# nicrie/xmca

Hardware: AMD Instinct MI355X
Metric: MCA solve+rotate throughput (ms_per_step = solve+rotate wall-clock, ms); rule_n surrogates/s in `rule_n` (higher is better)
Workload: dtype f64; 1 GPU; C2: synthetic EOF T=2920 x N=10000 float64 (generator A), solve() + rotate(n_rot=10, power=1); parallelism=replicas x1 (solve/rotate do not shard); rule_n run-sharded x1

## Files before the change

### xmca_amd/csrc/tridiag.h

```cpp
#pragma once
#include <algorithm>
#include <cmath>
#include <cstring>
#include <vector>

#include "common.h"

namespace xmca {

constexpr int TRD_THREADS = 512;
constexpr int TRD_ROWS = 4;
constexpr int TRD_MAX_WGS = 256;
constexpr int TRD_MAX_ITERS = 32;

struct TrdParams {
  double* Ar;
  double* Ai;
  int64_t ld;
  int n;
  double* vb[2][2];
  double* pb[2][2];
  double* gp[2][2];
  double* tau[2];
  double* d;
// ... 657 lines not shown
      if (is_writer && tid == 0) P.d[j] = dj_sh;
      break;
    }
    const double a0r = a0_sh[cur][0], a0i = CPLX ? a0_sh[cur][1] : 0.0;
    double beta, tr, ti = 0.0, scr = 0.0, sci = 0.0;
    if (xn2 == 0.0 && a0i == 0.0) {
      beta = a0r;
      tr = 0.0;
    } else {
      beta = -copysign(trd_sqrt(a0r * a0r + a0i * a0i + xn2), a0r);
      const double rb = trd_rcp(beta);
      tr = fma(fma(-(beta - a0r) * rb, beta, beta - a0r), rb, (beta - a0r) * rb);
      ti = -a0i * rb;
      const double dr = a0r - beta, di = a0i, dn = trd_rcp(dr * dr + di * di);
      scr = dr * dn;
      sci = -di * dn;
    }
    const double mr_ = trd_uniform(tr * scr - ti * sci), mi_ = trd_uniform(tr * sci + ti * scr);
    const double tr_next = trd_uniform(tr), ti_next = trd_uniform(ti), sr_next = trd_uniform(scr), si_next = trd_uniform(sci);
    if (is_writer && tid == 0) {
      P.d[j] = dj_sh;
      P.e[j] = beta;
      P.tau[0][j] = tr;
      if (CPLX) P.tau[1][j] = ti;
    }
    if (prof) P.prof[8 * j + 3] = __builtin_amdgcn_s_memtime();
    const int g0 = ((j + 1) >> 7) / CG;
    const int c0 = (j + 1) >> 7;
    if (lane == 0) bX[0][j + 1] = a0r - beta;
    const unsigned int tgn = trd_tag_of(j + 1);
    double* const xnext = reinterpret_cast<double*>(reinterpret_cast<char*>(S.xch) + xwr);
    auto publish_p = [&](int i, double pr, double pi) {
      if constexpr (CPLX) {
        trd_st16_sc1(S.xch, xbytes, 16 * i, xwr + xhalf, trd_tagged(pr, tgn), trd_tagged(pi, tgn));
      } else {
        trd_st_sc1(xnext + 2 * i + 1, trd_tagged(pr, tgn));
      }
    };
    {
      constexpr int MC = (NC + 3) / 4;
      int i = (int)blockIdx.x;
      if (i < j + 1) i += ((j + 1 - i + nwg - 1) / nwg) * nwg;
      int par = 0;
      for (; i < first_res; i += nwg, par ^= 1) {
        const double svr_ = bV[0][i], swr_ = bW[0][i];
        const double svi_ = CPLX ? bV[1][i] : 0.0, swi_ = CPLX ? bW[1][i] : 0.0;
        double* rowr = P.Ar + (int64_t)i * P.ld;
        double* rowi = CPLX ? P.Ai + (int64_t)i * P.ld : nullptr;
        double sr = 0.0, si = 0.0;
        const bool pubrow = i == j + 1;
#pragma unroll 1
        for (int u0 = 0; u0 < MC; u0 += 4) {
        double2 la[4], lb[4];
#pragma unroll
        for (int uu = 0; uu < 4; ++uu) {
          const int u = u0 + uu;
          const int c = u < MC ? c0 + wave + 4 * u : NC;
          la[uu] = make_double2(0.0, 0.0);
          lb[uu] = make_double2(0.0, 0.0);
          if (c < NC) {
            la[uu] = *reinterpret_cast<const double2*>(rowr + 128 * c + 2 * lane);
            if (CPLX) lb[uu] = *reinterpret_cast<const double2*>(rowi + 128 * c + 2 * lane);
          }
        }
#pragma unroll
        for (int uu = 0; uu < 4; ++uu) {
          const int u = u0 + uu;
          const int c = u < MC ? c0 + wave + 4 * u : NC;
          if (c < NC) {
            const int k = 128 * c + 2 * lane;
            double2 a = la[uu];
            const double2 wk = *reinterpret_cast<const double2*>(bW[0] + k);
            const double2 vk = *reinterpret_cast<const double2*>(bV[0] + k);
            const double2 xk = *reinterpret_cast<const double2*>(bX[0] + k);
            if (CPLX) {
              double2 b = lb[uu];
              const double2 wki = *reinterpret_cast<const double2*>(bW[1] + k);
              const double2 vki = *reinterpret_cast<const double2*>(bV[1] + k);
              const double2 xki = *reinterpret_cast<const double2*>(bX[1] + k);
              a.x -= (svr_ * wk.x + svi_ * wki.x) + (swr_ * vk.x + swi_ * vki.x);
              b.x -= (svi_ * wk.x - svr_ * wki.x) + (swi_ * vk.x - swr_ * vki.x);
              a.y -= (svr_ * wk.y + svi_ * wki.y) + (swr_ * vk.y + swi_ * vki.y);
              b.y -= (svi_ * wk.y - svr_ * wki.y) + (swi_ * vk.y - swr_ * vki.y);
              *reinterpret_cast<double2*>(rowr + k) = a;
              *reinterpret_cast<double2*>(rowi + k) = b;
              sr += a.x * xk.x - b.x * xki.x;
              si += a.x * xki.x + b.x * xk.x;
              sr += a.y * xk.y - b.y * xki.y;
              si += a.y * xki.y + b.y * xk.y;
              if (pubrow) {
                trd_st16_sc1(S.xch, xbytes, 16 * k, xwr, trd_tagged(a.x, tgn), trd_tagged(b.x, tgn));
                trd_st16_sc1(S.xch, xbytes, 16 * k + 16, xwr, trd_tagged(a.y, tgn), trd_tagged(b.y, tgn));
              }
            } else {
              a.x -= svr_ * wk.x + swr_ * vk.x;
              a.y -= svr_ * wk.y + swr_ * vk.y;
              *reinterpret_cast<double2*>(rowr + k) = a;
              sr += a.x * xk.x;
              sr += a.y * xk.y;
            }
            if (pubrow) {
              if constexpr (!CPLX) {
                trd_st_sc1(xnext + 2 * k, trd_tagged(a.x, tgn));
                trd_st_sc1(xnext + 2 * k + 2, trd_tagged(a.y, tgn));
              }
            }
          }
        }
        }
        sr = trd_wave_sum_dpp(sr);
        if (CPLX) si = trd_wave_sum_dpp(si);
        if (lane == 0) {
          rowpart[par][wave][0] = sr;
          rowpart[par][wave][1] = si;
        }
        __syncthreads();
        if (wave == 0) {
          const double yr = ((rowpart[par][0][0] + rowpart[par][1][0]) + rowpart[par][2][0]) + rowpart[par][3][0];
          const double yi = CPLX ? ((rowpart[par][0][1] + rowpart[par][1][1]) + rowpart[par][2][1]) + rowpart[par][3][1] : 0.0;
          const double pr = mr_ * yr - mi_ * yi, pi = mr_ * yi + mi_ * yr;
          if (lane == 0) publish_p(i, pr, pi);
        }
      }
    }
    if (rowi[RR - 1] > j) {
      double vpr[RR], vpi[RR], wpr[RR], wpi[RR], accr[RR], acci[RR];
#pragma unroll
      for (int t = 0; t < RR; ++t) {
        const int i = rowi[t];
        const int ii = i < n ? i : 0;
        vpr[t] = i < n ? bV[0][ii] : 0.0; wpr[t] = i < n ? bW[0][ii] : 0.0;
        vpi[t] = (CPLX && i < n) ? bV[1][ii] : 0.0; wpi[t] = (CPLX && i < n) ? bW[1][ii] : 0.0;
        accr[t] = 0.0; acci[t] = 0.0;
      }
#pragma unroll
      for (int cg = 0; cg < NC / CG; ++cg) {
        if (cg >= g0) {
#pragma unroll
          for (int cc = 0; cc < CG; ++cc) {
            const int c = cg * CG + cc;
            const int k = 128 * c + 2 * lane;
            const double2 wk = *reinterpret_cast<const double2*>(bW[0] + k);
            const double2 vk = *reinterpret_cast<const double2*>(bV[0] + k);
            const double2 xk = *reinterpret_cast<const double2*>(bX[0] + k);
            double2 wki = make_double2(0.0, 0.0), vki = wki, xki = wki;
            if (CPLX) {
              wki = *reinterpret_cast<const double2*>(bW[1] + k);
              vki = *reinterpret_cast<const double2*>(bV[1] + k);
              xki = *reinterpret_cast<const double2*>(bX[1] + k);
            }
#pragma unroll
            for (int t = 0; t < RR; ++t) {
              double2 a = ar[t][c];
              if (CPLX) {
                double2 b = ai[t][c];
                a.x = fma(-vpr[t], wk.x, a.x);  a.x = fma(-vpi[t], wki.x, a.x);  a.x = fma(-wpr[t], vk.x, a.x);  a.x = fma(-wpi[t], vki.x, a.x);
                b.x = fma(-vpi[t], wk.x, b.x);  b.x = fma(vpr[t], wki.x, b.x);   b.x = fma(-wpi[t], vk.x, b.x);  b.x = fma(wpr[t], vki.x, b.x);
                a.y = fma(-vpr[t], wk.y, a.y);  a.y = fma(-vpi[t], wki.y, a.y);  a.y = fma(-wpr[t], vk.y, a.y);  a.y = fma(-wpi[t], vki.y, a.y);
                b.y = fma(-vpi[t], wk.y, b.y);  b.y = fma(vpr[t], wki.y, b.y);   b.y = fma(-wpi[t], vk.y, b.y);  b.y = fma(wpr[t], vki.y, b.y);
                ai[t][c] = b;
                accr[t] = fma(a.x, xk.x, accr[t]);  accr[t] = fma(-b.x, xki.x, accr[t]);
                acci[t] = fma(a.x, xki.x, acci[t]); acci[t] = fma(b.x, xk.x, acci[t]);
                accr[t] = fma(a.y, xk.y, accr[t]);  accr[t] = fma(-b.y, xki.y, accr[t]);
                acci[t] = fma(a.y, xki.y, acci[t]); acci[t] = fma(b.y, xk.y, acci[t]);
              } else {
                a.x = fma(-vpr[t], wk.x, a.x);  a.x = fma(-wpr[t], vk.x, a.x);
                a.y = fma(-vpr[t], wk.y, a.y);  a.y = fma(-wpr[t], vk.y, a.y);
                accr[t] = fma(a.x, xk.x, accr[t]);
                accr[t] = fma(a.y, xk.y, accr[t]);
              }
              ar[t][c] = a;
            }
          }
          __builtin_amdgcn_sched_barrier(0);
        }
      }
#pragma unroll
      for (int t = 0; t < RR; ++t) {
        if (rowi[t] == j + 1) {
          int lane2 = 2 * lane;
          asm volatile("" : "+v"(lane2));
#pragma unroll
          for (int c = 0; c < NC; ++c) {
            if (c >= c0) {
              const int k = 128 * c + lane2;
              if constexpr (CPLX) {
                trd_st16_sc1(S.xch, xbytes, 16 * k, xwr, trd_tagged(ar[t][c].x, tgn), trd_tagged(ai[t][c].x, tgn));
                trd_st16_sc1(S.xch, xbytes, 16 * k + 16, xwr, trd_tagged(ar[t][c].y, tgn), trd_tagged(ai[t][c].y, tgn));
              } else {
                trd_st_sc1(xnext + 2 * k, trd_tagged(ar[t][c].x, tgn));
                trd_st_sc1(xnext + 2 * k + 2, trd_tagged(ar[t][c].y, tgn));
              }
            }
          }
        }
      }
      if (j + 1 == j_end && j_end < n) {
#pragma unroll
        for (int t = 0; t < RR; ++t) {
          if (rowi[t] > j && rowi[t] < n) {
            int lane2 = 2 * lane;
            asm volatile("" : "+v"(lane2));
            double* const dr_ = P.Ar + (int64_t)rowi[t] * P.ld;
            double* const di_ = CPLX ? P.Ai + (int64_t)rowi[t] * P.ld : nullptr;
#pragma unroll
            for (int c = 0; c < NC; ++c) {
              if (c >= c0) {
                const int k = 128 * c + lane2;
                *reinterpret_cast<double2*>(dr_ + k) = ar[t][c];
                if (CPLX) *reinterpret_cast<double2*>(di_ + k) = ai[t][c];
              }
            }
          }
        }
      }
#pragma unroll
      for (int t = 0; t < RR; ++t) {
        const int i = rowi[t];
        if (i < n && i > j) {
          const double yr = trd_wave_sum_dpp(accr[t]);
          const double yi = CPLX ? trd_wave_sum_dpp(acci[t]) : 0.0;
          const double pr = mr_ * yr - mi_ * yi, pi = mr_ * yi + mi_ * yr;
          if (lane == 0) publish_p(i, pr, pi);
        }
      }
    }
    if (prof) P.prof[8 * j + 4] = __builtin_amdgcn_s_memtime();
    __syncthreads();
    if (prof) P.prof[8 * j + 6] = __builtin_amdgcn_s_memtime();
    if (give_up_sh) {
      if (tid == 0) atomicExch(S.give_up, 1);
      break;
    }
    if (is_writer && j + 1 == j_end && j_end < n) {
      int s0 = tid;
      asm volatile("" : "+v"(s0));
      for (int s = s0; s < LV; s += TRD_RES_THREADS) {
        S.hand_u[0][s] = bX[0][s];
        if (CPLX) S.hand_u[1][s] = bX[1][s];
      }
      if (tid == 0) {
        S.hand_s[0] = tr_next; S.hand_s[1] = ti_next; S.hand_s[2] = sr_next; S.hand_s[3] = si_next;
      }
    }
    { double* t0 = bV[0]; bV[0] = bX[0]; bX[0] = t0; }
    if (CPLX) { double* t1 = bV[1]; bV[1] = bX[1]; bX[1] = t1; }
    tpr = tr_next;
    tpi = ti_next;
    spr = sr_next;
    spi = si_next;
  }
}

__global__ void trd_prefill_kernel(const double* __restrict__ Wr, const double* __restrict__ Wi, int n, double* __restrict__ xch) {
  const int k = blockIdx.x * blockDim.x + threadIdx.x;
  if (k >= n) return;
  if (Wi) {
    xch[2 * k] = trd_untagged(Wr[k]);
    xch[2 * k + 1] = trd_untagged(Wi[k]);
  } else {
    xch[2 * k] = trd_untagged(Wr[k]);
  }
}

__global__ __launch_bounds__(256) void trd_maxabs_kernel(const double* __restrict__ Ar, const double* __restrict__ Ai, int n, int64_t lda,
                                                         unsigned long long* __restrict__ acc) {
  double m = 0.0;
  bool bad = false;
  for (int r = blockIdx.x; r < n; r += gridDim.x)
    for (int c = threadIdx.x; c < n; c += 256) {
      const double a = fabs(Ar[(int64_t)r * lda + c]), b = Ai ? fabs(Ai[(int64_t)r * lda + c]) : 0.0;
      if (!(a <= 1.7e308) || !(b <= 1.7e308)) bad = true;
      m = fmax(m, fmax(a, b));
    }
  for (int o = 32; o > 0; o >>= 1) m = fmax(m, __shfl_xor(m, o));
  if (__any(bad)) { if ((threadIdx.x & 63) == 0) atomicOr(acc + 1, 1ull); }
  else if ((threadIdx.x & 63) == 0 && m > 0.0) atomicMax(acc, (unsigned long long)__double_as_longlong(m));
}
__global__ void trd_scale_kernel(const unsigned long long* __restrict__ acc, double* __restrict__ scal) {
  const double g = __longlong_as_double((long long)acc[0]);
  const bool nan = acc[1] != 0ull;
  double f = 1.0;
  if (g > 0.0 && !nan) {
    int ex;
    frexp(g, &ex);
    f = ldexp(1.0, -ex);
  }
  scal[0] = f;
  scal[1] = nan ? 1.0 : 0.0;
}

__global__ void trd_copy_kernel(const double* __restrict__ Ar, const double* __restrict__ Ai, int n, int64_t lda, double* Wr, double* Wi,
                                int64_t ld, const double* __restrict__ scal) {
  const double f = scal[0];
  const int r = blockIdx.x;
  for (int c = threadIdx.x; c < ld; c += blockDim.x) {
    const bool in = c < n;
    Wr[(int64_t)r * ld + c] = in ? f * Ar[(int64_t)r * lda + c] : 0.0;
    if (Wi) Wi[(int64_t)r * ld + c] = in ? f * Ai[(int64_t)r * lda + c] : 0.0;
  }
}

constexpr int TRD_BIS_THREADS = 256;
__global__ __launch_bounds__(TRD_BIS_THREADS) void trd_bisect_kernel(const double* __restrict__ d, const double* __restrict__ e, int n,
                                                                   const double* __restrict__ scal, double* lam_desc, double* lam_asc_scaled, int* flag) {
  extern __shared__ __attribute__((aligned(16))) double bis_lds[];
  __shared__ double red[2][TRD_BIS_THREADS / 64];
  double* sd = bis_lds;
  double* se2 = bis_lds + n;
  const int tid = threadIdx.x;
  double gl = 1.7e308, gu = -1.7e308;
  bool bad = false;
  for (int i = tid; i < n; i += TRD_BIS_THREADS) {
    const double di = d[i];
    const double el = i > 0 ? e[i - 1] : 0.0, er = i < n - 1 ? e[i] : 0.0;
    if (!(fabs(di) <= 1.7e308) || !(fabs(er) <= 1.7e308)) bad = true;
    sd[i] = di;
    se2[i] = fmax(er * er, 0x1p-200);
    const double r = fabs(el) + fabs(er);
    gl = fmin(gl, di - r);
    gu = fmax(gu, di + r);
  }
  for (int o = 32; o > 0; o >>= 1) {
    gl = fmin(gl, __shfl_xor(gl, o));
    gu = fmax(gu, __shfl_xor(gu, o));
  }
  if (__any(bad) && flag) { if ((tid & 63) == 0) atomicOr(flag, 1); }
  if ((tid & 63) == 0) { red[0][tid >> 6] = gl; red[1][tid >> 6] = gu; }
  __syncthreads();
  for (int w = 0; w < TRD_BIS_THREADS / 64; ++w) { gl = fmin(gl, red[0][w]); gu = fmax(gu, red[1][w]); }
  const double bnorm = fmax(fabs(gl), fabs(gu));
  gl -= 2.2e-16 * bnorm * n + 1e-300;
  gu += 2.2e-16 * bnorm * n + 1e-300;
  const int grp = tid >> 4, l = tid & 15;
  const int k = blockIdx.x * (TRD_BIS_THREADS / 16) + grp;
  const bool live = k < n;
  double lo = gl, hi = gu;
  const int gshift = ((tid & 63) >> 4) * 16;
  for (int pass = 0; pass < 14; ++pass) {
    const double x = lo + (hi - lo) * ((double)(l + 1) * (1.0 / 17.0));
    double pm = 1.0, pc = sd[0] - x;
    unsigned int sc = (unsigned int)__double2hiint(pc);
    int cnt = (int)(sc >> 31);
    int i = 1;
    double dv[8], ev[8];
    if (i + 8 <= n) {
#pragma unroll
      for (int u = 0; u < 8; ++u) { dv[u] = sd[i + u]; ev[u] = se2[i + u - 1]; }
    }
    for (; i + 8 <= n; i += 8) {
      double dn[8], en[8];
      const int inext = i + 16 <= n ? i + 8 : i;
#pragma unroll
      for (int u = 0; u < 8; ++u) { dn[u] = sd[inext + u]; en[u] = se2[inext + u - 1]; }
#pragma unroll
      for (int u = 0; u < 8; ++u) {
        const double pn = fma(dv[u] - x, pc, -(ev[u] * pm));
        const unsigned int sn = (unsigned int)__double2hiint(pn);
        cnt += (int)((sn ^ sc) >> 31);
        sc = sn;
        pm = pc;
        pc = pn;
      }
      const double mx = fmax(fabs(pc), fabs(pm));
      if (mx == 0.0) pc = (sc >> 31) ? -1.0 : 1.0;
      const int ex = __builtin_amdgcn_frexp_exp(mx);
      pc = ldexp(pc, -ex);
      pm = ldexp(pm, -ex);
#pragma unroll
      for (int u = 0; u < 8; ++u) { dv[u] = dn[u]; ev[u] = en[u]; }
    }
    for (; i < n; ++i) {
      const double pn = fma(sd[i] - x, pc, -(se2[i - 1] * pm));
      const unsigned int sn = (unsigned int)__double2hiint(pn);
      cnt += (int)((sn ^ sc) >> 31);
      sc = sn;
      pm = pc;
      pc = pn;
    }
    const unsigned long long mask = __ballot(cnt <= k);
    const int s = __popcll((mask >> gshift) & 0xFFFFull);
    const double x_lo = __shfl(x, s > 0 ? s - 1 : 0, 16);
    const double x_hi = __shfl(x, s < 16 ? s : 15, 16);
    if (s > 0) lo = x_lo;
    if (s < 16) hi = x_hi;
  }
  if (live && l == 0) {
    lam_desc[n - 1 - k] = 0.5 * (lo + hi) / scal[0];
    if (lam_asc_scaled) lam_asc_scaled[k] = 0.5 * (lo + hi);
  }
}

struct TrdWorkspace {
  DevBuf<double> W[2];
  DevBuf<double> V[2];
  DevBuf<double> vec;
  DevBuf<double> scal;
  DevBuf<int> flag;
  DevBuf<unsigned long long> prof;
  DevBuf<double> sync;
  DevBuf<unsigned int> flags;
  int resident_used = 0;
  int stages_used = 0;
  std::string last_desc;
  hipEvent_t ev[2] = {nullptr, nullptr};
  bool ev_pending = false;
  double reduce_ms = 0.0;
  long long reduce_calls = 0;
  long long resident_calls = 0;
  void ev_begin(hipStream_t st) {
    if (!ev[0]) { XMCA_HIP(hipEventCreate(&ev[0])); XMCA_HIP(hipEventCreate(&ev[1])); }
    XMCA_HIP(hipEventRecord(ev[0], st));
  }
  void ev_end(hipStream_t st) { XMCA_HIP(hipEventRecord(ev[1], st)); ev_pending = true; }
  void ev_collect() {
    if (!ev_pending) return;
    float t = 0.f;
    if (hipEventSynchronize(ev[1]) == hipSuccess && hipEventElapsedTime(&t, ev[0], ev[1]) == hipSuccess) { reduce_ms += t; ++reduce_calls; }
    ev_pending = false;
  }
  ~TrdWorkspace() { if (ev[0]) { (void)hipEventDestroy(ev[0]); (void)hipEventDestroy(ev[1]); } }
  double ms = 0.0;
};

inline bool trd_enabled() {
  const char* e = std::getenv("XMCA_TRIDIAG");
  return !(e && e[0] == '0');
}

inline size_t trd_step_lds(int n, bool cplx) { return (size_t)(((n + 3) + 1) & ~1) * 3 * (cplx ? 2 : 1) * sizeof(double); }

inline bool trd_fits(int n, bool cplx) {
  return trd_step_lds(n, cplx) + 8192 <= (size_t)160 * 1024 && n + 4 <= 16 * TRD_THREADS && (size_t)n * 16 <= (size_t)150 * 1024;
}

struct TrdLayout {
  int n;
  int64_t ld;
  size_t nv;
  double* base;
  TrdParams params(double* Wr, double* Wi, double* Vr, double* Vi) const {
    TrdParams P{};
    P.Ar = Wr; P.Ai = Wi; P.ld = ld; P.n = n;
    double* p = base;
    for (int a = 0; a < 2; ++a) for (int c = 0; c < 2; ++c) { P.vb[a][c] = p; p += nv; }
    for (int a = 0; a < 2; ++a) for (int c = 0; c < 2; ++c) { P.pb[a][c] = p; p += nv; }
    for (int a = 0; a < 2; ++a) for (int c = 0; c < 2; ++c) { P.gp[a][c] = p; p += TRD_MAX_WGS; }
    for (int c = 0; c < 2; ++c) { P.tau[c] = p; p += nv; }
    P.d = p; p += nv;
    P.e = p; p += nv;
    P.Vr = Vr; P.Vi = Vi;
    P.prof = nullptr;
    return P;
  }
  static size_t doubles(size_t nv) { return nv * 12 + (size_t)TRD_MAX_WGS * 8; }
};


inline int trd_resident_nc(int n, bool cplx) {
  const char* em = std::getenv("XMCA_TRD_RESIDENT_MIN_N");
  const int min_n = em ? std::atoi(em) : 384;
  const char* eo = std::getenv("XMCA_TRD_RESIDENT");
  const bool on = !(eo && eo[0] == '0');
  if (!on || n < min_n) return 0;
  if (n <= 8 * 128) return 8;
  if (n <= 16 * 128) return 16;
  if (cplx) return n <= 20 * 128 ? 20 : 0;
  return n <= 24 * 128 ? 24 : 0;
}

inline unsigned int trd_spin_limit() {
  static std::mutex mu;
  static std::map<int, int>* warm = new std::map<int, int>;
  int dev = 0;
  (void)hipGetDevice(&dev);
  std::lock_guard<std::mutex> lk(mu);
  return (*warm)[dev]++ == 0 ? (1u << 20) : (1u << 17);
}

struct TrdStage {
  int nc, rr;
  int col0;
  int j_begin, j_end;
};
inline int trd_stage_nc(int n, bool cplx) {
  for (int nc = 4; nc <= (cplx ? 20 : 24); nc += 4)
    if (n <= nc * 128) return nc;
  return 0;
}
inline int trd_stage_rr(int nc, bool cplx) { return cplx ? (nc <= 8 ? 1 : 2) : (nc + 7) / 8; }
inline int trd_stage_rr_packed(int nc, bool cplx) {
  if (!cplx) return trd_stage_rr(nc, cplx);
  if (nc == 12) return 3;
  if (nc == 8 || nc == 4) return 2;
  return trd_stage_rr(nc, cplx);
}
inline bool trd_pack_lanes() {
  const char* e = std::getenv("XMCA_TRD_PACK");
  return e ? e[0] != '0' : in_surrogate_lanes();
}
inline std::vector<TrdStage> trd_plan(int n, bool cplx, int nc) {
  std::vector<TrdStage> st;
  if (nc <= 0) return st;
  std::vector<int> cuts;
  const char* eb = std::getenv("XMCA_TRD_BREAKS");
  const char* ec = std::getenv("XMCA_TRD_CHAIN");
  const bool chain = !(ec && ec[0] == '0');
  if (chain) {
    if (eb && eb[0]) {
      for (const char* q = eb; *q;) {
        const int c = std::atoi(q);
        if (c > 0 && c % 256 == 0 && c < n - 256 && (cuts.empty() || c > cuts.back())) cuts.push_back(c);
        while (*q && *q != ',') ++q;
        if (*q == ',') ++q;
      }
    } else {
      for (int cnc = nc - 4; cnc >= 4; cnc -= 4) {
        const int cap = cnc * 128;
        if (n <= cap) continue;
        const int c = ((n - cap + 255) / 256) * 256;
        if (c < n - 256 && (cuts.empty() || c > cuts.back())) cuts.push_back(c);
      }
    }
  }
  int begin = 0;
  for (size_t q = 0; q <= cuts.size(); ++q) {
    const int end = q < cuts.size() ? cuts[q] : n;
    TrdStage sg{};
    sg.col0 = begin;
    sg.nc = (q == 0 && !chain) ? nc : trd_stage_nc(n - begin, cplx);
    sg.rr = (q > 0 && chain && trd_pack_lanes()) ? trd_stage_rr_packed(sg.nc, cplx) : trd_stage_rr(sg.nc, cplx);
    sg.j_begin = begin;
    sg.j_end = end;
    st.push_back(sg);
    begin = end;
  }
  return st;
}

inline TrdParams trd_reduce(hipStream_t st, TrdWorkspace& ws, const double* Ar, const double* Ai, int n, int64_t lda, bool keep_reflectors) {
  const bool cplx = Ai != nullptr;
  const int nc = trd_resident_nc(n, cplx);
  const std::vector<TrdStage> stages = trd_plan(n, cplx, nc);
  int64_t ld = std::max<int64_t>(((int64_t)n + 2 + 15) & ~(int64_t)15, (int64_t)nc * 128);
  for (const TrdStage& sg : stages) ld = std::max<int64_t>(ld, (int64_t)sg.col0 + (int64_t)sg.nc * 128);
  const size_t nv = (size_t)((n + 8 + 15) & ~15);
  ws.W[0].ensure((size_t)n * ld);
  if (cplx) ws.W[1].ensure((size_t)n * ld);
  if (keep_reflectors) {
    ws.V[0].ensure((size_t)n * ld);
    XMCA_HIP(hipMemsetAsync(ws.V[0].get(), 0, sizeof(double) * (size_t)n * ld, st));
    if (cplx) {
      ws.V[1].ensure((size_t)n * ld);
      XMCA_HIP(hipMemsetAsync(ws.V[1].get(), 0, sizeof(double) * (size_t)n * ld, st));
    }
  }
  ws.vec.ensure(TrdLayout::doubles(nv));
  ws.scal.ensure(4);
  ws.flag.ensure(4);
  XMCA_HIP(hipMemsetAsync(ws.vec.get(), 0, sizeof(double) * TrdLayout::doubles(nv), st));
  XMCA_HIP(hipMemsetAsync(ws.flag.get(), 0, sizeof(int) * 4, st));
  TrdLayout lay{n, ld, nv, ws.vec.get()};
  TrdParams P = lay.params(ws.W[0].get(), cplx ? ws.W[1].get() : nullptr, keep_reflectors ? ws.V[0].get() : nullptr,
                           (keep_reflectors && cplx) ? ws.V[1].get() : nullptr);
  {
    unsigned long long* acc = reinterpret_cast<unsigned long long*>(ws.scal.get() + 2);
    XMCA_HIP(hipMemsetAsync(acc, 0, 2 * sizeof(unsigned long long), st));
    hipLaunchKernelGGL(trd_maxabs_kernel, dim3(std::min(n, 1024)), dim3(256), 0, st, Ar, Ai, n, lda, acc);
    hipLaunchKernelGGL(trd_scale_kernel, dim3(1), dim3(1), 0, st, acc, ws.scal.get());
  }
  hipLaunchKernelGGL(trd_copy_kernel, dim3(n), dim3(256), 0, st, Ar, Ai, n, lda, P.Ar, P.Ai, ld, ws.scal.get());
  ws.resident_used = 0;

  if (nc > 0) {
    PersistGate& gate = persist_gate();
    const int n_cus = gate.n_cus;
    const size_t lv = (size_t)(ld > (int64_t)nc * 128 ? ld : (int64_t)nc * 128);
    const size_t rec = cplx ? 4 : 2;
    const size_t sync_doubles = 2 * lv + 8 + 2 * rec * lv;
    ws.sync.ensure(sync_doubles);
    ws.flags.ensure(4);
    XMCA_HIP(hipMemsetAsync(ws.sync.get(), 0, sizeof(double) * sync_doubles, st));
    XMCA_HIP(hipMemsetAsync(ws.flags.get(), 0, sizeof(unsigned int) * 4, st));
    TrdSync S{};
    double* q = ws.sync.get();
    for (int c = 0; c < 2; ++c) { S.hand_u[c] = q; q += lv; }
    S.hand_s = q; q += 8;
    S.xch = q;
    S.xch_pb = (int)(rec * lv * sizeof(double));
    S.contiguous = in_surrogate_lanes() ? 1 : 0;
    S.spin_limit = trd_spin_limit();
    hipLaunchKernelGGL(trd_prefill_kernel, dim3(ceil_div(n, 256)), dim3(256), 0, st, P.Ar, P.Ai, n, S.xch);
    S.give_up = reinterpret_cast<int*>(ws.flags.get());
    using ResFn = void (*)(TrdParams, TrdSync, int);
    auto pick = [&](int snc, int srr) -> ResFn {
      if (cplx) {
        switch (snc) {
          case 4: return srr == 2 ? trd_resident_kernel<true, 4, 2> : trd_resident_kernel<true, 4, 1>;
          case 8: return srr == 2 ? trd_resident_kernel<true, 8, 2> : trd_resident_kernel<true, 8, 1>;
          case 12: return srr == 3 ? trd_resident_kernel<true, 12, 3> : trd_resident_kernel<true, 12, 2>;
          case 16: return trd_resident_kernel<true, 16, 2>;
          default: return trd_resident_kernel<true, 20, 2>;
        }
      }
      switch (snc) {
        case 4: return trd_resident_kernel<false, 4, 1>;
        case 8: return trd_resident_kernel<false, 8, 1>;
        case 12: return trd_resident_kernel<false, 12, 2>;
        case 16: return trd_resident_kernel<false, 16, 2>;
        case 20: return trd_resident_kernel<false, 20, 3>;
        default: return trd_resident_kernel<false, 24, 3>;
      }
    };
    static const char* prof_file_r = std::getenv("XMCA_TRD_PROF");
    if (prof_file_r) {
      P.prof = ws.prof.ensure((size_t)8 * n);
      XMCA_HIP(hipMemsetAsync(P.prof, 0, sizeof(unsigned long long) * 8 * (size_t)n, st));
    }
    int gave_up = 0;
    {
      PersistGate::Claim claim(gate, n_cus);
      ws.ev_begin(st);
      for (size_t q = 0; q < stages.size(); ++q) {
        const TrdStage& sg = stages[q];
        const int c0 = sg.col0, ns = n - c0;
        const int64_t off = (int64_t)c0 * ld + c0;
        TrdParams Pq = P;
        Pq.n = ns;
        Pq.Ar = P.Ar + off;
        if (P.Ai) Pq.Ai = P.Ai + off;
        Pq.d = P.d + c0; Pq.e = P.e + c0;
        Pq.tau[0] = P.tau[0] + c0; Pq.tau[1] = P.tau[1] + c0;
        if (P.Vr) Pq.Vr = P.Vr + off;
        if (P.Vi) Pq.Vi = P.Vi + off;
        if (P.prof) Pq.prof = P.prof + (size_t)8 * c0;
        TrdSync Sq = S;
        Sq.hand_u[0] = S.hand_u[0] + c0; Sq.hand_u[1] = S.hand_u[1] + c0;
        Sq.xch = S.xch + 2 * (size_t)c0;
        Sq.j_begin = sg.j_begin - c0;
        Sq.j_end = sg.j_end - c0;
        Sq.cont = q > 0 ? 1 : 0;
        const int wgs = std::max(1, std::min(std::min(n_cus, TRD_MAX_WGS), ceil_div(ns, (TRD_RES_THREADS / 64) * sg.rr)));
        const int first_res = std::max(0, ns - wgs * (TRD_RES_THREADS / 64) * sg.rr);
        const size_t lds = (size_t)sg.nc * 128 * 3 * (cplx ? 2 : 1) * sizeof(double);
        ResFn fn = pick(sg.nc, sg.rr);
        XMCA_HIP(hipFuncSetAttribute(reinterpret_cast<const void*>(fn), hipFuncAttributeMaxDynamicSharedMemorySize, 150 * 1024));
        hipLaunchKernelGGL(fn, dim3(wgs), dim3(TRD_RES_THREADS), lds, st, Pq, Sq, first_res);
      }
      ws.ev_end(st);
      XMCA_HIP(hipGetLastError());
      int dbg[4] = {0};
      XMCA_HIP(hipMemcpyAsync(dbg, S.give_up, sizeof(dbg), hipMemcpyDeviceToHost, st));
      XMCA_HIP(hipStreamSynchronize(st));
      gave_up = dbg[0];
      if (gave_up && xmca_trace("giveup"))
        std::fprintf(stderr, "xmca: trd_resident_kernel: workgroup %d ran out of its spins at column %d of its launch (n = %d, %d launches)\n", dbg[3], dbg[2], n, (int)stages.size());
    }
    ws.stages_used = (int)stages.size();
    {
      std::string d = stages.size() > 1 ? "chain of " + std::to_string(stages.size()) + " persistent launches: " : "";
      for (size_t q = 0; q < stages.size(); ++q) {
        const TrdStage& sg = stages[q];
        d += (q ? " -> " : "") + std::string("trd_resident_kernel<") + (cplx ? "complex" : "real") + ",NC=" + std::to_string(sg.nc) + ",RR=" + std::to_string(sg.rr) +
             ",tagged> columns [" + std::to_string(sg.j_begin) + "," + std::to_string(sg.j_end) + ")";
      }
      ws.last_desc = d;
    }
    if (prof_file_r) {
      std::vector<unsigned long long> hp((size_t)8 * n);
      XMCA_HIP(hipMemcpy(hp.data(), P.prof, sizeof(unsigned long long) * hp.size(), hipMemcpyDeviceToHost));
      if (FILE* f = std::fopen(prof_file_r, "w")) {
        for (int j = 0; j < n; ++j) {
          for (int q = 0; q < 7; ++q) std::fprintf(f, "%llu ", hp[(size_t)8 * j + q] - (q ? hp[(size_t)8 * j] : (j ? hp[(size_t)8 * (j - 1)] : hp[0])));
          std::fprintf(f, "\n");
        }
        std::fclose(f);
      }
      P.prof = nullptr;
    }
    if (!gave_up) {
      ws.resident_used = 1;
      ++ws.resident_calls;
      ws.ev_collect();
      return P;
    }
    ws.ev_pending = false;
    ws.resident_used = 2;
    ++persist_giveups();
    if (xmca_trace("giveup")) std::fprintf(stderr, "xmca: trd_resident_kernel (n = %d) gave up - repeated with one launch per column\n", n);
    hipLaunchKernelGGL(trd_copy_kernel, dim3(n), dim3(256), 0, st, Ar, Ai, n, lda, P.Ar, P.Ai, ld, ws.scal.get());
    XMCA_HIP(hipMemsetAsync(ws.vec.get(), 0, sizeof(double) * TrdLayout::doubles(nv), st));
    if (keep_reflectors) {
      XMCA_HIP(hipMemsetAsync(ws.V[0].get(), 0, sizeof(double) * (size_t)n * ld, st));
      if (cplx) XMCA_HIP(hipMemsetAsync(ws.V[1].get(), 0, sizeof(double) * (size_t)n * ld, st));
    }
  }

  ws.last_desc = std::string("trd_step_kernel<") + (cplx ? "complex" : "real") + "> x " + std::to_string(n) + " launches (one per column)";
  const size_t lds = trd_step_lds(n, cplx);
  const int slots = ((n + 3) + 1) & ~1;
  const int ns = slots <= 2 * TRD_THREADS ? 2 : slots <= 4 * TRD_THREADS ? 4 : slots <= 8 * TRD_THREADS ? 8 : 16;
  using StepFn = void (*)(TrdParams, int, int);
  StepFn fn = nullptr;
  XMCA_CHECK(!cplx || ns <= 8, XMCA_ERR_UNSUPPORTED, "trd_reduce: complex problem too large for the LDS of a workgroup");
  if (cplx) fn = ns == 2 ? trd_step_kernel<true, 2> : ns == 4 ? trd_step_kernel<true, 4> : trd_step_kernel<true, 8>;
  else fn = ns == 2 ? trd_step_kernel<false, 2> : ns == 4 ? trd_step_kernel<false, 4> : ns == 8 ? trd_step_kernel<false, 8> : trd_step_kernel<false, 16>;
  XMCA_HIP(hipFuncSetAttribute(reinterpret_cast<const void*>(fn), hipFuncAttributeMaxDynamicSharedMemorySize, 150 * 1024));
  static const char* prof_file = std::getenv("XMCA_TRD_PROF");
  if (prof_file) {
    P.prof = ws.prof.ensure((size_t)8 * n);
    XMCA_HIP(hipMemsetAsync(P.prof, 0, sizeof(unsigned long long) * 8 * (size_t)n, st));
  }
  int wgs_prev = 1;
  ws.ev_begin(st);
  for (int j = 0; j < n; ++j) {
    const int m = n - j - 1;
    const int wgs = std::max(1, std::min(TRD_MAX_WGS, (m + TRD_ROWS - 1) / TRD_ROWS));
    hipLaunchKernelGGL(fn, dim3(wgs), dim3(TRD_THREADS), lds, st, P, j, wgs_prev);
    wgs_prev = wgs;
  }
  ws.ev_end(st);
  XMCA_HIP(hipGetLastError());
  if (prof_file) {
    std::vector<unsigned long long> hp((size_t)8 * n);
    XMCA_HIP(hipMemcpyAsync(hp.data(), P.prof, sizeof(unsigned long long) * hp.size(), hipMemcpyDeviceToHost, st));
    XMCA_HIP(hipStreamSynchronize(st));
    if (FILE* f = std::fopen(prof_file, "w")) {
      for (int j = 0; j < n; ++j) {
        for (int q = 0; q < 7; ++q) std::fprintf(f, "%llu ", hp[(size_t)8 * j + q] - (q ? hp[(size_t)8 * j] : 0ull));
        std::fprintf(f, "\n");
      }
      std::fclose(f);
    }
  }
  return P;
}

inline void trd_trace_checksums(hipStream_t st, const TrdParams& P, const double* Ar, int n, int64_t lda) {
  std::vector<double> in((size_t)n * lda), d(n), e(n);
  XMCA_HIP(hipStreamSynchronize(st));
  XMCA_HIP(hipMemcpy(in.data(), Ar, sizeof(double) * in.size(), hipMemcpyDeviceToHost));
  XMCA_HIP(hipMemcpy(d.data(), P.d, sizeof(double) * n, hipMemcpyDeviceToHost));
  XMCA_HIP(hipMemcpy(e.data(), P.e, sizeof(double) * n, hipMemcpyDeviceToHost));
  unsigned long long ci = 1469598103934665603ull, co = ci;
  for (int i = 0; i < n; ++i) for (int j = 0; j < n; ++j) { unsigned long long b; std::memcpy(&b, &in[(size_t)i * lda + j], 8); ci = (ci ^ b) * 1099511628211ull; }
  for (int i = 0; i < n; ++i) { unsigned long long b; std::memcpy(&b, &d[i], 8); co = (co ^ b) * 1099511628211ull; if (i + 1 < n) { std::memcpy(&b, &e[i], 8); co = (co ^ b) * 1099511628211ull; } }
  std::fprintf(stderr, "trdsum n=%d in=%016llx out=%016llx\n", n, ci, co);
  if (const char* dir = std::getenv("XMCA_TRD_DUMP_DIR")) {
    char name[512];
    std::snprintf(name, sizeof(name), "%s/de_%016llx_%016llx.bin", dir, ci, co);
    if (FILE* f0 = std::fopen(name, "rb")) std::fclose(f0);
    else if (FILE* f1 = std::fopen(name, "wb")) { std::fwrite(d.data(), 8, n, f1); std::fwrite(e.data(), 8, n, f1); std::fclose(f1); }
  }
}

inline void trd_eigenvalues(hipStream_t st, TrdWorkspace& ws, const TrdParams& P, std::vector<double>& lam_host, double* lam_dev,
                            DevBuf<double>& lam_tmp, double* lam_asc_scaled = nullptr) {
  const int n = P.n;
  double* out = lam_dev ? lam_dev : lam_tmp.ensure((size_t)n);
  XMCA_HIP(hipFuncSetAttribute(reinterpret_cast<const void*>(trd_bisect_kernel), hipFuncAttributeMaxDynamicSharedMemorySize, 150 * 1024));
  hipLaunchKernelGGL(trd_bisect_kernel, dim3(ceil_div(n, TRD_BIS_THREADS / 16)), dim3(TRD_BIS_THREADS), sizeof(double) * 2 * (size_t)n, st, P.d,
                     P.e, n, ws.scal.get(), out, lam_asc_scaled, ws.flag.get());
  XMCA_HIP(hipGetLastError());
  lam_host.resize((size_t)n);
  int flag = 0;
  double scal[2] = {1.0, 0.0};
  XMCA_HIP(hipMemcpyAsync(lam_host.data(), out, sizeof(double) * n, hipMemcpyDeviceToHost, st));
  XMCA_HIP(hipMemcpyAsync(&flag, ws.flag.get(), sizeof(int), hipMemcpyDeviceToHost, st));
  XMCA_HIP(hipMemcpyAsync(scal, ws.scal.get(), sizeof(double) * 2, hipMemcpyDeviceToHost, st));
  XMCA_HIP(hipStreamSynchronize(st));
  ws.ev_collect();
  XMCA_CHECK(flag == 0 && scal[1] == 0.0, XMCA_ERR_NUMERIC, "SVD failed. NaN entries may be the problem.");
}

}
```

Before: 37.66 solve+rotate/s.

## Split Sturm-count bisection into two half-chains per eigenvalue with interleaved LDS records

Each eigenvalue's Sturm sequence is now evaluated by 32 lanes: 16 run the recurrence forward over the top half of the tridiagonal and 16 run it backward over the bottom half. The two halves are joined through a determinant-style merge that uses shuffles, which halves the serial dependency chain length. The d and e^2 values are stored as interleaved double2 records with the bottom half reversed, and the inner loop is double-buffered with sched barriers plus a bit-packed sign count. This doubles the number of workgroups and lanes used per eigenvalue, and it risks subtle inertia-count errors at the join point. The main loop bound uses nb, not len, which looks deliberate for the unrolled part.

```diff
diff --git a/xmca_amd/csrc/tridiag.h b/xmca_amd/csrc/tridiag.h
--- a/xmca_amd/csrc/tridiag.h
+++ b/xmca_amd/csrc/tridiag.h
@@ -983,21 +983,26 @@
 }
 
 constexpr int TRD_BIS_THREADS = 256;
+constexpr int TRD_BIS_LANES = 32;
+constexpr double TRD_E2_FLOOR = 0x1p-200;
 __global__ __launch_bounds__(TRD_BIS_THREADS) void trd_bisect_kernel(const double* __restrict__ d, const double* __restrict__ e, int n,
                                                                    const double* __restrict__ scal, double* lam_desc, double* lam_asc_scaled, int* flag) {
   extern __shared__ __attribute__((aligned(16))) double bis_lds[];
   __shared__ double red[2][TRD_BIS_THREADS / 64];
-  double* sd = bis_lds;
-  double* se2 = bis_lds + n;
+  __shared__ double e2m_sh;
   const int tid = threadIdx.x;
+  const int m = n >> 1, nb = n - 1 - m;
+  double2* recs = reinterpret_cast<double2*>(bis_lds);
   double gl = 1.7e308, gu = -1.7e308;
   bool bad = false;
   for (int i = tid; i < n; i += TRD_BIS_THREADS) {
     const double di = d[i];
     const double el = i > 0 ? e[i - 1] : 0.0, er = i < n - 1 ? e[i] : 0.0;
     if (!(fabs(di) <= 1.7e308) || !(fabs(er) <= 1.7e308)) bad = true;
-    sd[i] = di;
-    se2[i] = fmax(er * er, 0x1p-200);
+    const double e2l = fmax(el * el, TRD_E2_FLOOR), e2r = fmax(er * er, TRD_E2_FLOOR);
+    if (i <= m) recs[i] = make_double2(di, e2l);
+    else recs[m + 1 + (n - 1 - i)] = make_double2(di, e2r);
+    if (i == m) e2m_sh = e2r;
     const double r = fabs(el) + fabs(er);
     gl = fmin(gl, di - r);
     gu = fmax(gu, di + r);
@@ -1013,63 +1018,83 @@
   const double bnorm = fmax(fabs(gl), fabs(gu));
   gl -= 2.2e-16 * bnorm * n + 1e-300;
   gu += 2.2e-16 * bnorm * n + 1e-300;
-  const int grp = tid >> 4, l = tid & 15;
-  const int k = blockIdx.x * (TRD_BIS_THREADS / 16) + grp;
+  const int grp = tid / TRD_BIS_LANES, l = tid & 15;
+  const bool back = (tid >> 4) & 1;
+  const int k = blockIdx.x * (TRD_BIS_THREADS / TRD_BIS_LANES) + grp;
   const bool live = k < n;
   double lo = gl, hi = gu;
-  const int gshift = ((tid & 63) >> 4) * 16;
+  const int gshift = ((tid & 63) / TRD_BIS_LANES) * TRD_BIS_LANES;
+  const double2* rec = recs + (back && nb > 0 ? m + 1 : 0);
+  const int len = back ? nb : m;
+  const double2 rj = recs[m];
+  const double e2m = e2m_sh;
   for (int pass = 0; pass < 14; ++pass) {
     const double x = lo + (hi - lo) * ((double)(l + 1) * (1.0 / 17.0));
-    double pm = 1.0, pc = sd[0] - x;
-    unsigned int sc = (unsigned int)__double2hiint(pc);
-    int cnt = (int)(sc >> 31);
+    double pm = len > 0 ? 1.0 : 0.0, pc = len > 0 ? rec[0].x - x : 1.0;
+    unsigned int sg = (unsigned int)__double2hiint(pc) >> 31;
+    int cnt = (int)sg;
+    auto row = [&](double2 r) __attribute__((always_inline)) {
+      const double pn = fma(r.x - x, pc, -(r.y * pm));
+      sg = __builtin_amdgcn_alignbit(sg, (unsigned int)__double2hiint(pn), 31);
+      pm = pc;
+      pc = pn;
+    };
     int i = 1;
-    double dv[8], ev[8];
-    if (i + 8 <= n) {
-#pragma unroll
-      for (int u = 0; u < 8; ++u) { dv[u] = sd[i + u]; ev[u] = se2[i + u - 1]; }
-    }
-    for (; i + 8 <= n; i += 8) {
-      double dn[8], en[8];
-      const int inext = i + 16 <= n ? i + 8 : i;
-#pragma unroll
-      for (int u = 0; u < 8; ++u) { dn[u] = sd[inext + u]; en[u] = se2[inext + u - 1]; }
-#pragma unroll
-      for (int u = 0; u < 8; ++u) {
-        const double pn = fma(dv[u] - x, pc, -(ev[u] * pm));
-        const unsigned int sn = (unsigned int)__double2hiint(pn);
-        cnt += (int)((sn ^ sc) >> 31);
-        sc = sn;
-        pm = pc;
-        pc = pn;
-      }
+    double2 va[8], vb[8];
+    auto load8 = [&](double2 (&v)[8], int i0) __attribute__((always_inline)) {
+#pragma unroll
+      for (int u = 0; u < 8; ++u) v[u] = rec[i0 + u];
+    };
+    auto block8 = [&](const double2 (&v)[8]) __attribute__((always_inline)) {
+#pragma unroll
+      for (int u = 0; u < 8; ++u) row(v[u]);
+      cnt += __popc((sg ^ (sg >> 1)) & 0xFFu);
       const double mx = fmax(fabs(pc), fabs(pm));
-      if (mx == 0.0) pc = (sc >> 31) ? -1.0 : 1.0;
+      if (mx == 0.0) pc = (sg & 1u) ? -1.0 : 1.0;
       const int ex = __builtin_amdgcn_frexp_exp(mx);
       pc = ldexp(pc, -ex);
       pm = ldexp(pm, -ex);
-#pragma unroll
-      for (int u = 0; u < 8; ++u) { dv[u] = dn[u]; ev[u] = en[u]; }
-    }
-    for (; i < n; ++i) {
-      const double pn = fma(sd[i] - x, pc, -(se2[i - 1] * pm));
-      const unsigned int sn = (unsigned int)__double2hiint(pn);
-      cnt += (int)((sn ^ sc) >> 31);
-      sc = sn;
-      pm = pc;
-      pc = pn;
-    }
-    const unsigned long long mask = __ballot(cnt <= k);
+    };
+    if (i + 8 <= nb) load8(va, i);
+    while (i + 8 <= nb) {
+      const bool more = i + 16 <= nb;
+      load8(vb, more ? i + 8 : i);
+      __builtin_amdgcn_sched_barrier(0);
+      block8(va);
+      i += 8;
+      if (!more) break;
+      load8(va, i + 16 <= nb ? i + 8 : i);
+      __builtin_amdgcn_sched_barrier(0);
+      block8(vb);
+      i += 8;
+    }
+    for (; i < len; ++i) {
+      row(rec[i]);
+      cnt += (int)((sg ^ (sg >> 1)) & 1u);
+    }
+    const double ext = fma(rj.x - x, pc, -(rj.y * pm));
+    const double o_pc = __shfl_xor(pc, 16), o_pm = __shfl_xor(pm, 16), o_ext = __shfl_xor(ext, 16);
+    const double f_pc = back ? o_pc : pc, f_ext = back ? o_ext : ext;
+    const double q_c = back ? pc : o_pc, q_m = back ? pm : o_pm;
+    const double det = fma(f_ext, q_c, -((e2m * f_pc) * q_m));
+    const int total = cnt + __shfl_xor(cnt, 16) + (int)(((unsigned int)(__double2hiint(det) ^ __double2hiint(f_pc) ^ __double2hiint(q_c))) >> 31);
+    const unsigned long long mask = __ballot(total <= k);
     const int s = __popcll((mask >> gshift) & 0xFFFFull);
     const double x_lo = __shfl(x, s > 0 ? s - 1 : 0, 16);
     const double x_hi = __shfl(x, s < 16 ? s : 15, 16);
     if (s > 0) lo = x_lo;
     if (s < 16) hi = x_hi;
   }
-  if (live && l == 0) {
+  if (live && (tid & (TRD_BIS_LANES - 1)) == 0) {
     lam_desc[n - 1 - k] = 0.5 * (lo + hi) / scal[0];
     if (lam_asc_scaled) lam_asc_scaled[k] = 0.5 * (lo + hi);
   }
+}
+inline void trd_bisect_launch(hipStream_t st, const double* d, const double* e, int n, const double* scal, double* lam_desc, double* lam_asc_scaled,
+                              int* flag) {
+  XMCA_HIP(hipFuncSetAttribute(reinterpret_cast<const void*>(trd_bisect_kernel), hipFuncAttributeMaxDynamicSharedMemorySize, 150 * 1024));
+  hipLaunchKernelGGL(trd_bisect_kernel, dim3(ceil_div(n, TRD_BIS_THREADS / TRD_BIS_LANES)), dim3(TRD_BIS_THREADS), sizeof(double) * 2 * (size_t)n, st,
+                     d, e, n, scal, lam_desc, lam_asc_scaled, flag);
 }
 
 struct TrdWorkspace {
@@ -1439,9 +1464,7 @@
                             DevBuf<double>& lam_tmp, double* lam_asc_scaled = nullptr) {
   const int n = P.n;
   double* out = lam_dev ? lam_dev : lam_tmp.ensure((size_t)n);
-  XMCA_HIP(hipFuncSetAttribute(reinterpret_cast<const void*>(trd_bisect_kernel), hipFuncAttributeMaxDynamicSharedMemorySize, 150 * 1024));
-  hipLaunchKernelGGL(trd_bisect_kernel, dim3(ceil_div(n, TRD_BIS_THREADS / 16)), dim3(TRD_BIS_THREADS), sizeof(double) * 2 * (size_t)n, st, P.d,
-                     P.e, n, ws.scal.get(), out, lam_asc_scaled, ws.flag.get());
+  trd_bisect_launch(st, P.d, P.e, n, ws.scal.get(), out, lam_asc_scaled, ws.flag.get());
   XMCA_HIP(hipGetLastError());
   lam_host.resize((size_t)n);
   int flag = 0;
```

New measurement: 38.22 solve+rotate/s, median of 6. 1.5% higher.
